# dnbaker/dashing

Measured on AMD Instinct MI355X. Metric: genome-pairs/sec, all-pairs HLL Jaccard (Ertl-MLE), N=10000 p=14, higher is better.
Workload: dtype u8/u32 popcount + f64 estimator; 1 GPU; BASELINE configs[2]: 10000 synthetic sketches, p=14 (16384 B each), all-pairs dist on MI355X; n_sketches=10000, p=14, k=31, estimator=ERTL_MLE

## Files before the change

dashing_amd/csrc/abi.hip:

```cpp
#include <algorithm>
#include <cstdlib>
#include <cstring>
#include <new>

#include "ctx.h"

using namespace dsh;

static hipError_t create_copy_stream(hipStream_t *s)
{
    int least = 0, greatest = 0;
    if (hipDeviceGetStreamPriorityRange(&least, &greatest) != hipSuccess) greatest = 0;
    if (const char *e = std::getenv("DSH_COPY_STREAM_PRIORITY")) greatest = std::atoi(e);
    return hipStreamCreateWithPriority(s, hipStreamNonBlocking, greatest);
}

extern "C" {

const char *dsh_backend_name(void) { return "hip:gfx950"; }

int dsh_abi_version(void) { return DSH_ABI_VERSION; }

int dsh_device_count(void)
{
// ... 1034 lines not shown
#ifdef DSH_WHATIF_MFMA
    if (!std::strcmp(name, "pair_mfma")) {
        c->pair_mfma = v != 0;
        return DSH_OK;
    }
#endif
    if (!std::strcmp(name, "finalize_stop")) {
        if (v < 0 || v > 4) return fail(c, DSH_EINVAL, "finalize_stop must be in [0,4]");
        if (v && !c->profiling) return fail(c, DSH_ESTATE, "finalize_stop needs dsh_set_profiling(ctx, 1)");
        c->finalize_stop = (int)v;
        return DSH_OK;
    }
    if (!std::strcmp(name, "finalize_timing")) {
        if (v && !c->profiling) return fail(c, DSH_ESTATE, "finalize_timing needs dsh_set_profiling(ctx, 1)");
        c->finalize_timing = v != 0;
        return DSH_OK;
    }
    if (!std::strcmp(name, "nsplit")) {
        if (v < 0 || v > 64) return fail(c, DSH_EINVAL, "nsplit must be in [0,64]");
        c->nsplit = (int)v;
        return DSH_OK;
    }
    if (!std::strcmp(name, "emax") || !std::strcmp(name, "elow")) {
        if (v < -1 || v > (int64_t)kMaxListSide) return fail(c, DSH_EINVAL, "%s must be in [-1,%u]", name, kMaxListSide);
        (name[1] == 'm' ? c->emax_opt : c->elow_opt) = (int)v;
        return DSH_OK;
    }
    if (!std::strcmp(name, "part_band_tiles")) {
        if (v < 1 || v > (1 << 30)) return fail(c, DSH_EINVAL, "part_band_tiles out of range");
        c->part_band_tiles = (int)v;
        return DSH_OK;
    }
    if (!std::strcmp(name, "xch_tail_bands")) {
        if (v < 0 || v > 8) return fail(c, DSH_EINVAL, "xch_tail_bands out of range");
        c->tail_bands = (int)v;
        return DSH_OK;
    }
    if (!std::strcmp(name, "overflow_frag_permille")) {
        if (v < 0 || v > 1000) return fail(c, DSH_EINVAL, "overflow_frag_permille out of range");
        c->overflow_frag_permille = (int)v;
        return DSH_OK;
    }
    if (!std::strcmp(name, "xch_recv_gate")) {
        if (v < -1 || v > 1) return fail(c, DSH_EINVAL, "xch_recv_gate is -1 (auto), 0 or 1");
        c->xch_recv_gate = (int)v;
        return DSH_OK;
    }
// ... 10 lines not shown
```

dashing_amd/csrc/consts.h:

```cpp
#pragma once
#include <stdint.h>

namespace dsh {

constexpr uint32_t kTile = 128;
constexpr uint32_t kListCap = 512;
constexpr uint32_t kMaxListSide = 255;
constexpr uint32_t kMaxBuckets = 1u << 15;
constexpr int kMaxPLds = 17;
constexpr int kMaxPReg32 = 15;
constexpr int kMaxPCompare = 24;
constexpr int kMaxP = 24;
constexpr uint32_t kThrChunk = 4096;
constexpr uint32_t kBandMaxRows = 1u << 20;
constexpr uint32_t kSketchSub = 8192;

}
```

dashing_amd/csrc/engine.hip:

```cpp
#include <algorithm>
#include <chrono>
#include <cstring>

#include "ctx.h"

namespace dsh {

int prepare(dsh_ctx *c, int estim, int want_sorted, bool card_only, uint64_t want_rb, uint64_t want_re, uint32_t nparts,
            int rowsorted, const std::vector<uint64_t> *extra_in)
{
    static const std::vector<uint64_t> kNoExtra;
    std::vector<uint64_t> extra_cached;
    const std::vector<uint64_t> *extra = extra_in ? extra_in : &kNoExtra;
    if (!c->have_sketches) return fail(c, DSH_ESTATE, "no sketches loaded");
    if (estim < 0 || estim > 2) return fail(c, DSH_EINVAL, "bad estimator %d", estim);
    if (want_sorted < 0) {
        want_sorted = c->lay.sorted;
        want_rb = c->lay.rb;
        want_re = c->lay.re;
        rowsorted = 0;
        extra_cached = c->lay.extra;
        extra = &extra_cached;
    }
    if (!want_sorted) rowsorted = 0, extra = &kNoExtra;
    if (want_re > c->n) want_re = c->n;
    if (!want_sorted) want_rb = 0, want_re = c->n;
    if (want_rb > want_re) want_rb = want_re;
    const uint64_t n = c->n;
    std::vector<uint64_t> parts, rs_pos;
    if (want_rb >= want_re) extra = &kNoExtra;
    if (want_sorted && !rowsorted) {
        if (extra->empty()) plan::range_parts(n, want_rb, want_re, std::max<uint32_t>(nparts, 1), parts);
        else parts = {want_rb, want_re};
    }
    if (rowsorted) plan::rowsorted_part_positions(n, want_rb, want_re, std::max<uint32_t>(nparts, 1), rs_pos, extra);
    const int emax_new = c->emax_opt >= 0 ? std::min<int>(c->emax_opt, (int)kMaxListSide) : plan::auto_list_cap(c->p, true);
    const int elow_new = c->elow_opt >= 0 ? std::min<int>(c->elow_opt, (int)kMaxListSide) : plan::auto_list_cap(c->p, false);
    if (emax_new != c->emax || elow_new != c->elow) {
        c->planes_valid = false;
        c->card_estim = -1;
    }
    c->emax = emax_new;
    c->elow = elow_new;
    const bool same_layout = c->planes_valid && c->lay_gen == c->pass_gen && c->lay.sorted == want_sorted &&
                             (!want_sorted || (c->lay.rb == want_rb && c->lay.re == want_re && c->lay.rowsorted == rowsorted &&
                                               c->lay.extra == *extra && (rowsorted ? c->lay.part_w == rs_pos : c->lay.parts == parts)));
    const uint64_t need_from = (card_only || !want_sorted || c->pass_from_zero) ? 0 : want_rb;
    const bool have_pass = c->card_estim == estim && c->card_from <= need_from;
    if (have_pass && (card_only || same_layout)) return DSH_OK;
    const bool keep_layout = same_layout && have_pass;
    hipEvent_t e0 = nullptr, e1 = nullptr;
    if (c->profiling) {
        e0 = next_event(c);
        e1 = next_event(c);
        if (e0) (void)hipEventRecord(e0, c->stream);
    }
    if (!have_pass) {
        HIPCHK(c, c->card.ensure(std::max<uint64_t>(n, 1) * sizeof(double)));
        HIPCHK(c, c->exc.ensure(std::max<uint64_t>(n, 1) * kListCap * (c->p <= 15 ? 2 : 4)));
        HIPCHK(c, c->excv.ensure(std::max<uint64_t>(n, 1) * kListCap));
        HIPCHK(c, c->exc_n.ensure(std::max<uint64_t>(n, 1) * sizeof(uint32_t)));
        HIPCHK(c, c->keys.ensure(std::max<uint64_t>(n, 1) * sizeof(uint32_t)));
        HIPCHK(c, c->tailhist.ensure(std::max<uint64_t>(n, 1) * 64));
        HIPCHK(c, c->hist.ensure(std::max<uint64_t>(n, 1) * 64 * sizeof(uint32_t)));
        HIPCHK(c, launch_selfhist_card(c->stream, c->regs, need_from, n, c->p, estim, c->emax, c->elow,
                                       (uint32_t *)c->hist.ptr, c->exc.ptr, (uint8_t *)c->excv.ptr,
                                       (uint32_t *)c->exc_n.ptr, (uint32_t *)c->keys.ptr,
                                       (uint8_t *)c->tailhist.ptr));
        HIPCHK(c, c->pin_keys.ensure(std::max<uint64_t>(n, 1) * sizeof(uint32_t)));
        c->hk32 = (const uint32_t *)c->pin_keys.ptr;
        if (n > need_from)
            HIPCHK(c, hipMemcpyAsync((uint32_t *)c->pin_keys.ptr + need_from, (const uint32_t *)c->keys.ptr + need_from,
                                     (n - need_from) * sizeof(uint32_t), hipMemcpyDeviceToHost, c->stream));
        if (!c->ev_keys) HIPCHK(c, hipEventCreateWithFlags(&c->ev_keys, hipEventDisableTiming));
        HIPCHK(c, hipEventRecord(c->ev_keys, c->stream));
        HIPCHK(c, launch_card_from_hist(c->stream, (const uint32_t *)c->hist.ptr, (const uint32_t *)c->keys.ptr, need_from, n,
                                        c->p, estim, (double *)c->card.ptr));
        c->card_estim = estim;
        c->card_from = need_from;
        c->hk32_valid = false;
        ++c->pass_gen;
    }
    if (card_only) {
// ... 509 lines not shown
```

dashing_amd/csrc/host/plan_capi.cpp:

```cpp
#include <algorithm>
#include <cstdarg>
#include <cstdio>
#include <cstring>
#include <vector>

#include "../plan.h"
#include "../uf.h"

using namespace dsh;
using namespace dsh::plan;

namespace {

struct Err {
    char *buf;
    size_t cap;
    int fail(const char *fmt, ...)
    {
        if (buf && cap) {
            va_list ap;
            va_start(ap, fmt);
            vsnprintf(buf, cap, fmt, ap);
            va_end(ap);
        }
// ... 377 lines not shown
        ++nb;
    }
    return (int64_t)nb;
}

int dsh_plan_uf_labels(uint64_t n, const uint32_t *lhs, const uint32_t *rhs, uint64_t n_edges, uint32_t step_cap, uint32_t *labels_out)
{
    if (n > 0xFFFFFFFFull) return -1;
    std::vector<uint32_t> parent(n);
    for (uint64_t x = 0; x < n; ++x) parent[x] = (uint32_t)x;
    for (uint64_t e = 0; e < n_edges; ++e) {
        if (lhs[e] >= n || rhs[e] >= n) return -1;
        uint32_t why = 0;
        if (uf_unite<UfPlain>(parent.data(), lhs[e], rhs[e], step_cap, &why) == kUfOverrun) return (int)why;
    }
    for (uint64_t x = 0; x < n; ++x) {
        const uint32_t l = uf_find<UfPlain>(parent.data(), (uint32_t)x, step_cap);
        if (l == kUfOverrun) return (int)kUfErrFind;
        labels_out[x] = l;
    }
    return 0;
}

}
```

dashing_amd/csrc/kernels.h:

```cpp
#pragma once
#include <hip/hip_runtime.h>
#include <stdint.h>

#include "consts.h"

namespace dsh {

hipError_t launch_selfhist_card(hipStream_t st, const uint8_t *regs, uint64_t first, uint64_t n, int p, int estim,
                                int emax, int elow, uint32_t *hist, void *exc, uint8_t *excv, uint32_t *exc_n,
                                uint32_t *keys, uint8_t *tailhist);
hipError_t launch_card_from_hist(hipStream_t st, const uint32_t *hist, const uint32_t *keys, uint64_t first, uint64_t n, int p,
                                 int estim, double *card);
inline int colindex_inline(int p, uint32_t E) { return p <= 12 && E <= 256 ? 7 : 3; }
struct ColIndexLaunch {
    const void *exc;
    const uint8_t *excv;
    const uint32_t *exc_n, *keys;
    const double *card;
    const uint8_t *tailhist;
    const uint32_t *perm;
    uint64_t ncols;
    int p;
    uint32_t nblocks, nbuckets, ent_stride, E;
    uint32_t *rec;
    uint32_t *ent;
    uint32_t *nS, *keyS;
    double *cardS;
    uint8_t *thS;
    uint32_t *rl;
};
hipError_t launch_build_colindex(hipStream_t st, const ColIndexLaunch &c);
hipError_t launch_transform(hipStream_t st, const uint8_t *regs, uint64_t n, int p, int vlo,
                            uint32_t P, uint32_t W, uint32_t Npad, uint32_t *planes,
                            const uint32_t *perm);
hipError_t launch_pair_counts(hipStream_t st, int kc, int cum_bytes, const uint32_t *planes,
                              uint32_t Npad, uint32_t Kpad, uint32_t W, uint32_t P,
// ... 216 lines not shown
```

dashing_amd/csrc/kernels_compare.hip:

```cpp
#include <hip/hip_runtime.h>
#include <stdint.h>

#include <algorithm>

#include "estimators.h"
#include "kernels.h"

namespace dsh {

template <typename PT>
__global__ __launch_bounds__(256, 4) void k_selfhist_card(const uint8_t *__restrict__ regs, uint64_t first,
                                                        uint64_t n, int p, int estim, int emax, int elow,
                                                        uint32_t *__restrict__ hist_out,
                                                        PT *__restrict__ exc,
                                                        uint8_t *__restrict__ excv,
                                                        uint32_t *__restrict__ exc_n,
                                                        uint32_t *__restrict__ keys,
                                                        uint8_t *__restrict__ tailhist)
{
    __shared__ uint32_t hist[4][64];
    __shared__ uint32_t sub[4][8][72];
    __shared__ int thr[4], thrL[4];
    const int tid = threadIdx.x, lane = tid & 63, wave = tid >> 6;
    const uint64_t s = first + (uint64_t)blockIdx.x * 4 + wave;
#pragma unroll
    for (int k = 0; k < 8; ++k) sub[wave][k][lane] = 0;
    __syncthreads();
    const uint64_t m = 1ull << p;
    const uint4 *src = reinterpret_cast<const uint4 *>(regs + (s < n ? s : 0) * m);
    const uint64_t nch = m >> 4;
    constexpr int kRegCache = 16;
    uint4 cache[kRegCache];
#pragma unroll
    for (int k = 0; k < kRegCache; ++k) {
        const uint64_t c = (uint64_t)k * 64 + lane;
// ... 36 lines not shown
        while (lo < 63 && h[lo] == 0) ++lo;
        while (hi > 0 && h[hi] == 0) --hi;
        int T = hi;
        uint32_t cnt = 0;
        while (T > lo && cnt + h[T] <= (uint32_t)emax) {
            cnt += h[T];
            --T;
        }
        int L = lo;
        uint32_t cntl = 0;
        while (L < T && cntl + h[L] <= (uint32_t)elow) {
            cntl += h[L];
            ++L;
        }
        thr[wave] = T;
        thrL[wave] = L;
        exc_n[s] = cnt + cntl;
        keys[s] = ((uint32_t)hi << 18) | ((uint32_t)T << 12) | ((uint32_t)L << 6) | (uint32_t)lo;
    }
    if (s < n && __any(bad != 0) && lane == 0) atomicOr(&keys[s], 0x80000000u);
    __syncthreads();
    if (s >= n) return;
    const uint32_t T = (uint32_t)thr[wave], L = (uint32_t)thrL[wave];
    tailhist[s * 64 + lane] = (uint32_t)lane > T ? (uint8_t)hist[wave][lane] : (uint8_t)0;
    hist_out[s * 64 + lane] = hist[wave][lane];
    if (emax == 0 && elow == 0) return;
    PT *dstp = exc + s * kListCap;
    uint8_t *dstv = excv + s * kListCap;
    const uint32_t trep = (T + 1) * 0x01010101u, lrep = L * 0x01010101u;
    auto hits = [trep, lrep](uint32_t x) -> uint32_t {
        const uint32_t ge = ((x | 0x80808080u) - trep) & 0x80808080u;
        const uint32_t lt = ~((x | 0x80808080u) - lrep) & 0x80808080u;
        return ge | lt;
    };
    uint32_t mine = 0;
#pragma unroll
    for (int k = 0; k < kRegCache; ++k)
        if ((uint64_t)k * 64 + lane < nch) {
            const uint32_t w[4] = {cache[k].x, cache[k].y, cache[k].z, cache[k].w};
#pragma unroll
            for (int q = 0; q < 4; ++q) mine += (uint32_t)__popc(hits(w[q]));
        }
    for (uint64_t c = (uint64_t)kRegCache * 64 + lane; c < nch; c += 64) {
        const uint4 x = src[c];
        mine += (uint32_t)(__popc(hits(x.x)) + __popc(hits(x.y)) + __popc(hits(x.z)) + __popc(hits(x.w)));
    }
    uint32_t slot = mine;
#pragma unroll
    for (int d = 1; d < 64; d <<= 1) {
        const uint32_t o = __shfl_up(slot, d, 64);
        if (lane >= d) slot += o;
    }
    slot -= mine;
    auto emit4 = [&](uint32_t x, uint32_t pos0) {
        uint32_t h = hits(x);
        while (h) {
            const uint32_t b = (uint32_t)__builtin_ctz(h) >> 3;
            h &= h - 1;
            if (slot < kListCap) {
                dstp[slot] = (PT)(pos0 + b);
                dstv[slot] = (uint8_t)((x >> (8 * b)) & 0xFFu);
            }
            ++slot;
        }
    };
#pragma unroll
    for (int k = 0; k < kRegCache; ++k) {
        const uint64_t c = (uint64_t)k * 64 + lane;
        if (c < nch) {
            const uint32_t w[4] = {cache[k].x, cache[k].y, cache[k].z, cache[k].w};
#pragma unroll
            for (int q = 0; q < 4; ++q) emit4(w[q], (uint32_t)(c * 16 + q * 4));
        }
    }
    for (uint64_t c = (uint64_t)kRegCache * 64 + lane; c < nch; c += 64) {
        const uint4 x = src[c];
        emit4(x.x, (uint32_t)(c * 16));
        emit4(x.y, (uint32_t)(c * 16 + 4));
        emit4(x.z, (uint32_t)(c * 16 + 8));
        emit4(x.w, (uint32_t)(c * 16 + 12));
    }
}
// ... 19 lines not shown
__global__ __launch_bounds__(1024) void k_build_colindex(const PT *__restrict__ exc, const uint8_t *__restrict__ excv,
                                                          const uint32_t *__restrict__ exc_n,
                                                          const uint32_t *__restrict__ keys, const double *__restrict__ card,
                                                          const uint8_t *__restrict__ tailhist,
                                                          const uint32_t *__restrict__ perm, uint64_t ncols, int p,
                                                          uint32_t nbuckets, uint32_t ent_stride, uint32_t E,
                                                          uint32_t *__restrict__ rec, uint32_t *__restrict__ ent,
                                                          uint32_t *__restrict__ nS, uint32_t *__restrict__ keyS,
                                                          double *__restrict__ cardS, uint8_t *__restrict__ thS,
                                                          uint32_t *__restrict__ rl)
{
    extern __shared__ __attribute__((aligned(16))) uint32_t cnt[];
    __shared__ uint32_t part[1024];
    __shared__ uint32_t below_s;
    constexpr uint32_t RW = (uint32_t)RK + 1u;
    const uint32_t tid = threadIdx.x, lane = tid & 63u, wave = tid >> 6;
    const uint32_t sh = p > 14 ? (uint32_t)(p - 14) : 0u;
    const uint64_t c0 = (uint64_t)blockIdx.x * kTile;
    const uint32_t G = gridDim.y, g = blockIdx.y;
    const uint32_t nown = nbuckets / G, blo = g * nown;
    for (uint32_t b = tid; b < nown; b += 1024) cnt[b] = 0;
    if (tid == 0) below_s = 0;
    __syncthreads();
    constexpr int kPer = (int)(kListCap / 64);
    constexpr int kSk = (int)(kTile / 16);
    uint32_t Ts[kSk], pk[kSk][kPer];
    uint32_t sk[kSk], nes[kSk];
#pragma unroll
    for (int q = 0; q < kSk; ++q) {
        const uint64_t col = c0 + wave + 16u * (uint32_t)q;
        sk[q] = col < ncols ? (perm ? perm[col] : (uint32_t)col) : 0xFFFFFFFFu;
    }
#pragma unroll
    for (int q = 0; q < kSk; ++q) {
        nes[q] = sk[q] != 0xFFFFFFFFu ? exc_n[sk[q]] : 0u;
        Ts[q] = keys[sk[q] != 0xFFFFFFFFu ? sk[q] : 0u];
    }
#pragma unroll
    for (int q = 0; q < kSk; ++q) {
        const uint32_t sl = wave + 16u * (uint32_t)q;
        const bool ok = sk[q] != 0xFFFFFFFFu;
        const uint64_t s = ok ? sk[q] : 0;
        const uint32_t ne = nes[q];
        const uint32_t key = Ts[q];
        Ts[q] = (key >> 12) & 63u;
        const PT *ps = exc + s * kListCap;
        const uint8_t *vs = excv + s * kListCap;
        const uint64_t col = c0 + sl;
        const bool mine = (uint32_t)q % G == g;
        if (mine && lane == 0) {
            nS[col] = ne;
            keyS[col] = ok ? key : 0u;
            cardS[col] = ok ? card[s] : 0.;
        }
        if (mine && lane < 16) reinterpret_cast<uint32_t *>(thS + col * 64)[lane] = ok ? reinterpret_cast<const uint32_t *>(tailhist + s * 64)[lane] : 0u;
        uint32_t pos[kPer], val[kPer];
#pragma unroll
        for (int u = 0; u < kPer; ++u) {
            pos[u] = (uint32_t)ps[lane + 64u * (uint32_t)u];
            val[u] = (uint32_t)vs[lane + 64u * (uint32_t)u];
        }
#pragma unroll
        for (int u = 0; u < kPer; ++u) {
            const uint32_t e = lane + 64u * (uint32_t)u;
            pk[q][u] = e < ne ? ((pos[u] << 8) | val[u]) : 0xFFFFFFFFu;
            if (e < E && mine) rl[col * E + e] = pk[q][u];
        }
        __builtin_amdgcn_sched_barrier(0);
    }
    auto bucket_of = [sh](uint32_t x, uint32_t T) -> uint32_t {
        return x == 0xFFFFFFFFu ? x : ((((x >> 8) >> sh) << 1) | ((x & 0xFFu) > T ? 0u : 1u));
    };
    uint32_t below = 0;
#pragma unroll
    for (int q = 0; q < kSk; ++q)
#pragma unroll
        for (int u = 0; u < kPer; ++u) {
            const uint32_t b = bucket_of(pk[q][u], Ts[q]);
            const uint32_t rel = b - blo;
            if (rel < nown) atomicAdd(&cnt[rel], 1u);
            else if (b < blo) ++below;
        }
    if (G > 1) {
#pragma unroll
        for (int d = 32; d >= 1; d >>= 1) below += __shfl_xor(below, d, 64);
        if (lane == 0 && below) atomicAdd(&below_s, below);
    }
    __syncthreads();
    const uint32_t per = (nown + 1023) / 1024;
    uint32_t sum = 0;
    for (uint32_t b = tid * per; b < (tid + 1) * per && b < nown; ++b) sum += cnt[b];
    uint32_t incl = sum;
#pragma unroll
    for (int d = 1; d < 64; d <<= 1) {
        const uint32_t o = __shfl_up(incl, d, 64);
        if ((int)lane >= d) incl += o;
    }
    if (lane == 63) part[wave] = incl;
    __syncthreads();
    uint32_t wbase = 0;
    for (uint32_t w = 0; w < wave; ++w) wbase += part[w];
    uint32_t run = below_s + wbase + incl - sum;
    uint32_t *myrec = rec + ((uint64_t)blockIdx.x * nbuckets + blo) * RW;
    for (uint32_t b = tid * per; b < (tid + 1) * per && b < nown; ++b) {
        const uint32_t x = cnt[b];
        uint4 *r4 = reinterpret_cast<uint4 *>(myrec + (uint64_t)b * RW);
        r4[0] = make_uint4(x | (run << 16), 0xFFFFFFFFu, 0xFFFFFFFFu, 0xFFFFFFFFu);
        if constexpr (RK > 3) r4[1] = make_uint4(0xFFFFFFFFu, 0xFFFFFFFFu, 0xFFFFFFFFu, 0xFFFFFFFFu);
        cnt[b] = (run << 16) | run;
        run += x;
    }
    __syncthreads();
    uint32_t *myent = ent + (uint64_t)blockIdx.x * ent_stride;
#pragma unroll
    for (int q = 0; q < kSk; ++q)
#pragma unroll
        for (int u = 0; u < kPer; ++u)
        {
            uint32_t x = pk[q][u];
            asm volatile("" : "+v"(x));
            const uint32_t b = bucket_of(x, Ts[q]) - blo;
            if (b < nown) {
                const uint32_t pv = ((((x >> 8) & ((1u << sh) - 1u)) << 13) | ((wave + 16u * (uint32_t)q) << 6) | (x & 0xFFu));
                const uint32_t w = atomicAdd(&cnt[b], 1u);
                const uint32_t slot = w & 0xFFFFu, rel = slot - (w >> 16);
                myent[slot] = pv;
                if (rel < (uint32_t)RK) myrec[(uint64_t)b * RW + 1u + rel] = pv;
            }
        }
}

__device__ __forceinline__ uint32_t lt_word(const uint32_t (&y)[8], uint32_t vrep)
{
    uint32_t ge = 0;
#pragma unroll
    for (int k = 0; k < 8; ++k) ge |= ((y[k] - vrep) >> (7 - k)) & (0x01010101u << k);
    return ~ge;
}

__global__ __launch_bounds__(256) void k_transform(const uint8_t *__restrict__ regs, uint64_t n,
                                                    int p, int vlo, uint32_t P, uint32_t W,
                                                    uint32_t Npad, uint32_t *__restrict__ planes,
                                                    const uint32_t *__restrict__ perm)
{
    const uint64_t gid = (uint64_t)blockIdx.x * 256 + threadIdx.x;
    const uint32_t i = (uint32_t)(gid % Npad);
    const uint32_t w = (uint32_t)(gid / Npad);
    if (w >= W) return;
    const uint64_t m = 1ull << p;
    uint32_t x[8];
#pragma unroll
    for (int k = 0; k < 8; ++k) x[k] = 0xFFFFFFFFu;
// ... 503 lines not shown
{
    unsigned long long tph[7] = {0, 0, 0, 0, 0, 0, 0};
    if constexpr (TIMED) tph[0] = __builtin_readcyclecounter();
    extern __shared__ __attribute__((aligned(16))) unsigned char hs_raw[];
    uint32_t *histA = reinterpret_cast<uint32_t *>(hs_raw);
    uint32_t *corr = histA + 64;
    uint32_t *actm = corr + 128;
    CT *hs = reinterpret_cast<CT *>(hs_raw + (64 + 128 + 8) * 4);
    constexpr uint32_t RW = (uint32_t)RK + 1u;
    constexpr uint32_t kNone = 0xFFFFFFFFu;
    const int tid = threadIdx.x;
    const uint32_t kq = blockIdx.x >> 3;
    const uint32_t tidx = ((kq >> 7) << 3) + (blockIdx.x & 7u), trow = kq & 127u;
    if (tidx >= a.ntiles) return;
    uint4 tile = a.tiles[tidx];
    const int vlo = (int)((tile.z >> 16) & 0xFFu), vhi = (int)(tile.z >> 24);
    const uint32_t slot = ((tile.w & 0xFFFFu) * 128u + trow) * 128u + (uint32_t)tid;
    tile.w = (tile.z >> 8) & 0xFFu;
    tile.z &= 0xFFu;
    const uint32_t si = tile.x * kTile + trow;
    const uint32_t sj = tile.y * kTile + (uint32_t)tid;
    if (si >= a.ncols) return;
    const int Lp = a.pbase + (int)tile.z, T = a.pbase + (int)tile.w;
    constexpr int kR = RK > 3 ? 2 : (int)(kListCap / 128);
    const int nr = (int)((a.E + 127u) >> 7);
    uint32_t le[kR];
    {
        const uint32_t *rli = a.rl + (uint64_t)si * a.E;
#pragma unroll
        for (int r = 0; r < kR; ++r) {
            le[r] = kNone;
            if (r >= nr) continue;
            const uint32_t e = (uint32_t)tid + 128u * (uint32_t)r;
            if (e < a.E) le[r] = rli[e];
        }
    }
    const uint32_t i = a.perm ? (uint32_t)__builtin_amdgcn_readfirstlane((int)a.perm[si]) : si;
    const bool col_ok = sj < a.ncols;
    const uint32_t j = col_ok ? (a.perm ? a.perm[sj] : sj) : 0u;
    const CT *cum0 = reinterpret_cast<const CT *>(a.cum);
    constexpr int kBatch = 16;
    const int npl = (int)(tile.w - tile.z);
    uint32_t cvv[kBatch];
    const int w0 = (T + 1) >> 4;
    uint4 tq[3];
    {
        const CT *cp = cum0 + (uint64_t)tile.z * a.nslots;
#pragma unroll
        for (int t = 0; t < kBatch; ++t) {
            cvv[t] = 0u;
            if (t < npl) {
                cvv[t] = (uint32_t)cp[slot];
                cp += a.nslots;
                asm volatile("" : "+s"(cp));
            }
        }
    }
    {
        const uint4 *tb = reinterpret_cast<const uint4 *>(a.thS) + (sj << 2);
#pragma unroll
        for (int k = 0; k < 3; ++k) tq[k] = w0 + k < 4 ? tb[w0 + k] : make_uint4(0, 0, 0, 0);
    }
    const uint32_t keyj = a.keyS[sj];
    const uint32_t keyi = (uint32_t)__builtin_amdgcn_readfirstlane((int)a.keyS[si]);
    const uint32_t hrow = tid < 64 ? (uint32_t)(a.thS + (uint64_t)si * 64)[tid] : 0u;
    const uint32_t sh = a.p > 14 ? (uint32_t)(a.p - 14) : 0u;
    const uint32_t *brec = a.cidx_rec + (uint64_t)tile.y * a.nbuckets * RW;
    const uint32_t *bent = a.cidx_ent + (uint64_t)tile.y * a.ent_stride;
    const uint32_t rb32 = (uint32_t)a.row_begin, re32 = (uint32_t)a.row_end;
    const bool m_rect = GENERAL && a.rect, m_square = GENERAL && a.square, m_sorted = GENERAL && a.sorted_out, m_knn = GENERAL && a.knn;
    if (m_rect && !(i >= rb32 && i < re32)) return;
    corr[tid] = 0;
    if (tid < 64) histA[tid] = tid > T ? hrow : 0u;
    {
        uint32_t nup = 0;
#pragma unroll
        for (int r = 0; r < kR; ++r) {
            if (r >= nr) break;
            nup += (uint32_t)__popcll(__ballot(le[r] != kNone && (int)(le[r] & 0xFFu) > T));
        }
        if ((tid & 63) == 0) actm[4 + (tid >> 6)] = nup;
    }
    uint32_t oi = i, oj = j;
    bool active;
    if (m_rect) {
        active = j >= (uint32_t)a.col_begin && j < (uint32_t)a.col_end;
    } else if (m_square) {
        active = si < sj;
    } else if (m_sorted || m_knn) {
        oi = si;
        oj = sj;
// ... 36 lines not shown
                prev = cvv[t];
            }
        }
        for (uint32_t pl = tile.z + kBatch; pl < tile.w; ++pl) {
            const uint32_t cv = (cum0 + (uint64_t)pl * a.nslots)[slot];
            dcol[pl * 128] = (CT)(cv - prev);
            prev = cv;
        }
    }
    uint4 rc[kR], rc2[RK > 3 ? kR : 1];
#pragma unroll
    for (int r = 0; r < kR; ++r) {
        rc[r] = make_uint4(0u, kNone, kNone, kNone);
        if constexpr (RK > 3) rc2[r] = make_uint4(kNone, kNone, kNone, kNone);
        if (r >= nr) continue;
        const int va = (int)(le[r] & 0xFFu);
        const bool up = va > T;
        if (le[r] == kNone || !(up || va < Lp)) continue;
        const uint32_t bk = (((le[r] >> 8) >> sh) << 1) | (up ? 0u : 1u);
        const uint4 *rp = reinterpret_cast<const uint4 *>(brec + (uint64_t)bk * RW);
        rc[r] = rp[0];
        if constexpr (RK > 3) rc2[r] = rp[1];
    }
    if (active) {
        const uint32_t qw[12] = {tq[0].x, tq[0].y, tq[0].z, tq[0].w, tq[1].x, tq[1].y, tq[1].z, tq[1].w,
                                 tq[2].x, tq[2].y, tq[2].z, tq[2].w};
        const int x0 = w0 * 16;
        CT *dst = col + (x0 - vlo) * 128;
        const uint32_t *hA = histA + x0;
#pragma unroll
        for (int s_ = 0; s_ < 48; ++s_) {
            const int x = x0 + s_;
            if (x > vhi) break;
            if (x <= T) continue;
            const uint32_t qj = (qw[s_ >> 2] >> (8 * (s_ & 3))) & 0xFFu;
            nb += qj;
            dst[s_ * 128] = (CT)(hA[s_] + qj);
        }
        for (int x = x0 + 48; x <= vhi; ++x) {
            const uint32_t qj = a.thS[(uint64_t)sj * 64 + x];
            nb += qj;
            col[(x - vlo) * 128] = (CT)(histA[x] + qj);
        }
    }
    __syncthreads();
    if constexpr (TIMED) tph[2] = __builtin_readcyclecounter();
    if (a.stop == 2) {
        const FinalizeArgs *L = &a;
        if (active) L->out[out_index(L)] = (float)(nb + prev + keyj);
        return;
    }
    {
        uint32_t *hw = reinterpret_cast<uint32_t *>(hs);
        const bool all_own = (actm[0] & actm[1] & actm[2] & actm[3]) == 0xFFFFFFFFu;
        auto apply = [&](uint32_t x, int var, bool upr, uint32_t plow) {
            const uint32_t jl = (x >> 6) & 127u;
            const int vb = (int)(x & 63u);
            if (x == kNone || (sh && (x >> 13) != plow) || !(upr ? vb > T : vb < Lp)) return;
            if (!all_own && !((actm[jl >> 5] >> (jl & 31u)) & 1u)) return;
            const int bin = upr ? (var < vb ? var : vb) : (var > vb ? var : vb);
            const uint32_t cell = (uint32_t)(bin - vlo) * 128u + jl;
            const uint32_t one = sizeof(CT) == 2 ? 1u << (16u * (cell & 1u)) : 1u;
            uint32_t *w = &hw[sizeof(CT) == 2 ? cell >> 1 : cell];
            if (upr) {
                atomicAdd(&corr[jl], 1u);
                atomicSub(w, one);
            } else {
                atomicAdd(w, one);
            }
        };
#pragma unroll
        for (int r = 0; r < kR; ++r) {
            if (r >= nr) break;
            if (__ballot(rc[r].y != kNone) == 0) continue;
            const int va = (int)(le[r] & 0xFFu);
            const bool up = va > T;
            const uint32_t plow = (le[r] >> 8) & ((1u << sh) - 1u);
            apply(rc[r].y, va, up, plow);
            apply(rc[r].z, va, up, plow);
            apply(rc[r].w, va, up, plow);
            if constexpr (RK > 3) {
                apply(rc2[r].x, va, up, plow);
                apply(rc2[r].y, va, up, plow);
                apply(rc2[r].z, va, up, plow);
                apply(rc2[r].w, va, up, plow);
            }
            const uint32_t cnt = rc[r].x & 0xFFFFu, q0 = rc[r].x >> 16;
            for (uint32_t q = (uint32_t)RK; q < cnt; ++q) apply(bent[q0 + q], va, up, plow);
        }
    }
    __syncthreads();
    if constexpr (TIMED) tph[3] = __builtin_readcyclecounter();
    if (!active) return;
    const uint32_t ucnt = actm[4] + actm[5] + nb - corr[tid];
    uint32_t clow = 0;
    for (int x = vlo; x < Lp; ++x) clow += col[(x - vlo) * 128];
    if (tile.w > tile.z) col[(Lp - vlo) * 128] -= (CT)clow;
    else prev = clow;
    col[(T - vlo) * 128] = (CT)(m - ucnt - prev);
    if (a.stop == 3) {
        const FinalizeArgs *L = &a;
        L->out[out_index(L)] = (float)(ucnt + clow);
        return;
    }
    const int loj = (int)(keyj & 63u), loi = (int)(keyi & 63u);
    const int minv = loi > loj ? loi : loj;
    const int maxj = (int)((keyj >> 18) & 63u), maxi = (int)((keyi >> 18) & 63u);
    int maxv = maxi > maxj ? maxi : maxj;
    if (maxv < T) maxv = T;
    auto c = [col, vlo, vhi](int v) -> uint32_t {
        return (v < vlo || v > vhi) ? 0u : col[(v - vlo) * 128];
// ... 405 lines not shown
    uint64_t most = 0;
    for (uint32_t i = 0; i < nseg; ++i) most = std::max(most, u.s[i].nwords);
    if (!nseg || !most) return hipSuccess;
    const uint32_t blocks = (uint32_t)std::min<uint64_t>(256, (most + 255) / 256);
    hipLaunchKernelGGL(k_upload_segs, dim3(blocks, nseg), dim3(256), 0, st, u);
    return hipGetLastError();
}

hipError_t launch_upload(hipStream_t st, void *dst, const void *src_pinned, size_t bytes)
{
    if (bytes == 0) return hipSuccess;
    const uint64_t nwords = (bytes + 3) / 4;
    const uint32_t blocks = (uint32_t)std::min<uint64_t>(256, (nwords + 255) / 256);
    hipLaunchKernelGGL(k_upload, dim3(blocks), dim3(256), 0, st, (uint32_t *)dst, (const uint32_t *)src_pinned, nwords);
    return hipGetLastError();
}

hipError_t launch_selfhist_card(hipStream_t st, const uint8_t *regs, uint64_t first, uint64_t n, int p, int estim,
                                int emax, int elow, uint32_t *hist, void *exc, uint8_t *excv, uint32_t *exc_n,
                                uint32_t *keys, uint8_t *tailhist)
{
    if (n <= first) return hipSuccess;
    const uint32_t blocks = (uint32_t)((n - first + 3) / 4);
    if (p <= 15)
        hipLaunchKernelGGL(k_selfhist_card<uint16_t>, dim3(blocks), dim3(256), 0, st, regs, first, n, p, estim, emax, elow,
                           hist, (uint16_t *)exc, excv, exc_n, keys, tailhist);
    else
        hipLaunchKernelGGL(k_selfhist_card<uint32_t>, dim3(blocks), dim3(256), 0, st, regs, first, n, p, estim, emax, elow,
                           hist, (uint32_t *)exc, excv, exc_n, keys, tailhist);
    return hipGetLastError();
}

hipError_t launch_card_from_hist(hipStream_t st, const uint32_t *hist, const uint32_t *keys, uint64_t first, uint64_t n, int p,
                                 int estim, double *card)
{
    if (n <= first) return hipSuccess;
    hipLaunchKernelGGL(k_card_from_hist, dim3((uint32_t)((n - first + 63) / 64)), dim3(64), 0, st, hist, keys, first, n, p, estim, card);
    return hipGetLastError();
}

hipError_t launch_build_colindex(hipStream_t st, const ColIndexLaunch &c)
{
    if (c.nblocks == 0) return hipSuccess;
    uint32_t G = 1;
    while (G < 4 && c.nblocks * G < 256 && c.nbuckets / (2 * G) >= 4096) G *= 2;
    const size_t lds = (size_t)(c.nbuckets / G) * sizeof(uint32_t);
#define DSH_COLINDEX(PT, RK)                                                                                                  \
    do {                                                                                                                      \
        hipError_t e = ensure_dynamic_lds(reinterpret_cast<const void *>(k_build_colindex<PT, RK>), lds);                     \
        if (e != hipSuccess) return e;                                                                                        \
        hipLaunchKernelGGL((k_build_colindex<PT, RK>), dim3(c.nblocks, G), dim3(1024), lds, st, (const PT *)c.exc, c.excv,    \
// ... 145 lines not shown
```

dashing_amd/csrc/plan.cpp:

```cpp
#include "plan.h"

#include <algorithm>
#include <cstring>

namespace dsh {
namespace plan {

uint64_t tri_index(uint64_t n, uint64_t i, uint64_t j) { return i * (2 * n - i - 1) / 2 + j - (i + 1); }

uint64_t tri_span(uint64_t n, uint64_t rb, uint64_t re)
{
    if (re > n) re = n;
    if (rb >= re) return 0;
    const uint64_t cnt = re - rb;
    return cnt * (n - 1) - (rb + re - 1) * cnt / 2;
}

uint64_t tri_band_end(uint64_t n, uint64_t b0, uint64_t re, uint64_t band_floats, uint64_t row_cap)
{
    const uint64_t max_rows = std::min<uint64_t>(std::max<uint64_t>(row_cap, 1), kBandMaxRows);
    uint64_t b1 = b0, span = 0;
    do {
        span += n - 1 - b1;
        ++b1;
// ... 72 lines not shown

void range_parts(uint64_t n, uint64_t rb, uint64_t re, uint32_t nparts, std::vector<uint64_t> &out)
{
    out.assign(1, rb);
    if (re > n) re = n;
    if (rb > re) rb = re, out[0] = rb;
    const uint64_t total = tri_span(n, rb, re);
    for (uint32_t q = 1; q < nparts && out.back() < re; ++q) {
        const long double target = (long double)total * q / nparts;
        uint64_t best = out.back() + kTile;
        for (uint64_t cand = out.back() + kTile; cand < re; cand += kTile) {
            best = cand;
            if ((long double)tri_span(n, rb, cand) >= target) break;
        }
        if (best >= re) break;
        out.push_back(best);
    }
    if (out.back() != re) out.push_back(re);
}

int auto_list_cap(int p, bool upper)
{
    const uint64_t m = 1ull << p;
    return (int)std::min<uint64_t>(upper ? kMaxListSide : 200, m >> 5);
}

bool rowsorted_rule(uint64_t n, uint64_t rb, uint64_t re, uint32_t nparts)
{
    if (re > n) re = n;
    if (nparts < 2 || rb >= re) return false;
    return re - rb < (uint64_t)1024 * nparts && tri_span(n, rb, re) * sizeof(float) <= ((uint64_t)1 << 30);
}

uint64_t rowsorted_split(uint64_t n, uint64_t rb, uint64_t re)
{
    if (re > n) re = n;
    if (rb >= re) return re;
    const uint64_t TR = (re - rb + kTile - 1) / kTile, NTc = (n - rb + kTile - 1) / kTile;
    if (TR < 16) return re;
    uint64_t total = 0;
    for (uint64_t t = 0; t < TR; ++t) total += NTc - t;
    uint64_t K = 0, acc = 0;
    while (K < TR && acc * 100 < total * 15) acc += NTc - (TR - 1 - K), ++K;
    if (K < 2 || TR - K < 8) return re;
    const uint64_t x = rb + (TR - K) * kTile;
    const long double len_all = (long double)n - 1 - 0.5L * (long double)(rb + re - 1), len_tail = (long double)n - 1 - 0.5L * (long double)(x + re - 1);
    return len_tail <= 0.65L * len_all ? x : re;
// ... 830 lines not shown
```

Baseline: 3.924 billion pairs/s.

## Allow longer exception lists with chunked column-index build and extended tail histogram

Raises the upper exception-list cap (auto 312 at p=14, up to 1023 by option), sizing per-sketch list storage in 512-entry chunks. The column-index build streams extra chunks from global memory, and the compare kernel software-pipelines the extra rounds. The tail histogram packs overflow counts above 255 into its last bytes. The intent is to cover more pairs exactly through the sparse list path so fewer fall back to the dense slow path. In exchange each pair does more per-pair list work, memory use grows, and the count/offset bit packing changes.

```diff
diff --git a/dashing_amd/csrc/abi.hip b/dashing_amd/csrc/abi.hip
--- a/dashing_amd/csrc/abi.hip
+++ b/dashing_amd/csrc/abi.hip
@@ -1080,7 +1080,8 @@
         return DSH_OK;
     }
     if (!std::strcmp(name, "emax") || !std::strcmp(name, "elow")) {
-        if (v < -1 || v > (int64_t)kMaxListSide) return fail(c, DSH_EINVAL, "%s must be in [-1,%u]", name, kMaxListSide);
+        const uint32_t lim = name[1] == 'm' ? kMaxListUpper : kMaxListLower;
+        if (v < -1 || v > (int64_t)lim) return fail(c, DSH_EINVAL, "%s must be in [-1,%u]", name, lim);
         (name[1] == 'm' ? c->emax_opt : c->elow_opt) = (int)v;
         return DSH_OK;
     }
diff --git a/dashing_amd/csrc/consts.h b/dashing_amd/csrc/consts.h
--- a/dashing_amd/csrc/consts.h
+++ b/dashing_amd/csrc/consts.h
@@ -4,8 +4,11 @@
 namespace dsh {
 
 constexpr uint32_t kTile = 128;
-constexpr uint32_t kListCap = 512;
-constexpr uint32_t kMaxListSide = 255;
+constexpr uint32_t kListChunk = 512;
+constexpr uint32_t kMaxListUpper = 1023;
+constexpr uint32_t kMaxListLower = 255;
+constexpr int kMaxPLongList = 20;
+constexpr uint32_t list_cap(uint32_t E) { return E <= kListChunk ? kListChunk : (E + kListChunk - 1) / kListChunk * kListChunk; }
 constexpr uint32_t kMaxBuckets = 1u << 15;
 constexpr int kMaxPLds = 17;
 constexpr int kMaxPReg32 = 15;
diff --git a/dashing_amd/csrc/engine.hip b/dashing_amd/csrc/engine.hip
--- a/dashing_amd/csrc/engine.hip
+++ b/dashing_amd/csrc/engine.hip
@@ -34,8 +34,9 @@
         else parts = {want_rb, want_re};
     }
     if (rowsorted) plan::rowsorted_part_positions(n, want_rb, want_re, std::max<uint32_t>(nparts, 1), rs_pos, extra);
-    const int emax_new = c->emax_opt >= 0 ? std::min<int>(c->emax_opt, (int)kMaxListSide) : plan::auto_list_cap(c->p, true);
-    const int elow_new = c->elow_opt >= 0 ? std::min<int>(c->elow_opt, (int)kMaxListSide) : plan::auto_list_cap(c->p, false);
+    const int emax_lim = c->p <= kMaxPLongList ? (int)kMaxListUpper : 255;
+    const int emax_new = std::min<int>(c->emax_opt >= 0 ? c->emax_opt : plan::auto_list_cap(c->p, true), emax_lim);
+    const int elow_new = c->elow_opt >= 0 ? std::min<int>(c->elow_opt, (int)kMaxListLower) : plan::auto_list_cap(c->p, false);
     if (emax_new != c->emax || elow_new != c->elow) {
         c->planes_valid = false;
         c->card_estim = -1;
@@ -57,8 +58,9 @@
     }
     if (!have_pass) {
         HIPCHK(c, c->card.ensure(std::max<uint64_t>(n, 1) * sizeof(double)));
-        HIPCHK(c, c->exc.ensure(std::max<uint64_t>(n, 1) * kListCap * (c->p <= 15 ? 2 : 4)));
-        HIPCHK(c, c->excv.ensure(std::max<uint64_t>(n, 1) * kListCap));
+        const uint64_t lcap = list_cap((uint32_t)(c->emax + c->elow));
+        HIPCHK(c, c->exc.ensure(std::max<uint64_t>(n, 1) * lcap * (c->p <= 15 ? 2 : 4)));
+        HIPCHK(c, c->excv.ensure(std::max<uint64_t>(n, 1) * lcap));
         HIPCHK(c, c->exc_n.ensure(std::max<uint64_t>(n, 1) * sizeof(uint32_t)));
         HIPCHK(c, c->keys.ensure(std::max<uint64_t>(n, 1) * sizeof(uint32_t)));
         HIPCHK(c, c->tailhist.ensure(std::max<uint64_t>(n, 1) * 64));
diff --git a/dashing_amd/csrc/host/plan_capi.cpp b/dashing_amd/csrc/host/plan_capi.cpp
--- a/dashing_amd/csrc/host/plan_capi.cpp
+++ b/dashing_amd/csrc/host/plan_capi.cpp
@@ -423,4 +423,6 @@
     return 0;
 }
 
-}
+int dshh_auto_list_cap(int p, int upper) { return dsh::plan::auto_list_cap(p, upper != 0); }
+
+}
diff --git a/dashing_amd/csrc/kernels.h b/dashing_amd/csrc/kernels.h
--- a/dashing_amd/csrc/kernels.h
+++ b/dashing_amd/csrc/kernels.h
@@ -12,6 +12,8 @@
 hipError_t launch_card_from_hist(hipStream_t st, const uint32_t *hist, const uint32_t *keys, uint64_t first, uint64_t n, int p,
                                  int estim, double *card);
 inline int colindex_inline(int p, uint32_t E) { return p <= 12 && E <= 256 ? 7 : 3; }
+constexpr uint32_t cidx_count_bits(int p) { return p <= kMaxPLongList ? 14u : 16u; }
+constexpr int kTailExtMinP = 9;
 struct ColIndexLaunch {
     const void *exc;
     const uint8_t *excv;
diff --git a/dashing_amd/csrc/kernels_compare.hip b/dashing_amd/csrc/kernels_compare.hip
--- a/dashing_amd/csrc/kernels_compare.hip
+++ b/dashing_amd/csrc/kernels_compare.hip
@@ -2,6 +2,7 @@
 #include <stdint.h>
 
 #include <algorithm>
+#include <type_traits>
 
 #include "estimators.h"
 #include "kernels.h"
@@ -10,7 +11,7 @@
 
 template <typename PT>
 __global__ __launch_bounds__(256, 4) void k_selfhist_card(const uint8_t *__restrict__ regs, uint64_t first,
-                                                        uint64_t n, int p, int estim, int emax, int elow,
+                                                        uint64_t n, int p, int estim, int emax, int elow, uint32_t cap,
                                                         uint32_t *__restrict__ hist_out,
                                                         PT *__restrict__ exc,
                                                         uint8_t *__restrict__ excv,
@@ -93,11 +94,23 @@
     __syncthreads();
     if (s >= n) return;
     const uint32_t T = (uint32_t)thr[wave], L = (uint32_t)thrL[wave];
-    tailhist[s * 64 + lane] = (uint32_t)lane > T ? (uint8_t)hist[wave][lane] : (uint8_t)0;
+    {
+        const uint32_t hv = (uint32_t)lane > T ? hist[wave][lane] : 0u;
+        uint32_t byte = hv & 0xFFu;
+        if (p >= kTailExtMinP) {
+            unsigned long long big = __ballot(hv > 0xFFu);
+            if (lane >= 61) {
+                for (int k = 61; k < lane; ++k) big &= big - 1;
+                const int v = big ? __builtin_ctzll(big) : 0;
+                byte = big ? ((uint32_t)v << 2) | ((hist[wave][v] >> 8) & 3u) : 0u;
+            }
+        }
+        tailhist[s * 64 + lane] = (uint8_t)byte;
+    }
     hist_out[s * 64 + lane] = hist[wave][lane];
     if (emax == 0 && elow == 0) return;
-    PT *dstp = exc + s * kListCap;
-    uint8_t *dstv = excv + s * kListCap;
+    PT *dstp = exc + s * cap;
+    uint8_t *dstv = excv + s * cap;
     const uint32_t trep = (T + 1) * 0x01010101u, lrep = L * 0x01010101u;
     auto hits = [trep, lrep](uint32_t x) -> uint32_t {
         const uint32_t ge = ((x | 0x80808080u) - trep) & 0x80808080u;
@@ -128,7 +141,7 @@
         while (h) {
             const uint32_t b = (uint32_t)__builtin_ctz(h) >> 3;
             h &= h - 1;
-            if (slot < kListCap) {
+            if (slot < cap) {
                 dstp[slot] = (PT)(pos0 + b);
                 dstv[slot] = (uint8_t)((x >> (8 * b)) & 0xFFu);
             }
@@ -194,8 +207,11 @@
     for (uint32_t b = tid; b < nown; b += 1024) cnt[b] = 0;
     if (tid == 0) below_s = 0;
     __syncthreads();
-    constexpr int kPer = (int)(kListCap / 64);
+    constexpr int kPer = (int)(kListChunk / 64);
     constexpr int kSk = (int)(kTile / 16);
+    const uint32_t cap = list_cap(E);
+    const uint32_t nch = cap / kListChunk;
+    const uint32_t cb = cidx_count_bits(p);
     uint32_t Ts[kSk], pk[kSk][kPer];
     uint32_t sk[kSk], nes[kSk];
 #pragma unroll
@@ -208,98 +224,154 @@
         nes[q] = sk[q] != 0xFFFFFFFFu ? exc_n[sk[q]] : 0u;
         Ts[q] = keys[sk[q] != 0xFFFFFFFFu ? sk[q] : 0u];
     }
-#pragma unroll
-    for (int q = 0; q < kSk; ++q) {
-        const uint32_t sl = wave + 16u * (uint32_t)q;
-        const bool ok = sk[q] != 0xFFFFFFFFu;
-        const uint64_t s = ok ? sk[q] : 0;
-        const uint32_t ne = nes[q];
-        const uint32_t key = Ts[q];
-        Ts[q] = (key >> 12) & 63u;
-        const PT *ps = exc + s * kListCap;
-        const uint8_t *vs = excv + s * kListCap;
-        const uint64_t col = c0 + sl;
-        const bool mine = (uint32_t)q % G == g;
-        if (mine && lane == 0) {
-            nS[col] = ne;
-            keyS[col] = ok ? key : 0u;
-            cardS[col] = ok ? card[s] : 0.;
-        }
-        if (mine && lane < 16) reinterpret_cast<uint32_t *>(thS + col * 64)[lane] = ok ? reinterpret_cast<const uint32_t *>(tailhist + s * 64)[lane] : 0u;
-        uint32_t pos[kPer], val[kPer];
-#pragma unroll
-        for (int u = 0; u < kPer; ++u) {
-            pos[u] = (uint32_t)ps[lane + 64u * (uint32_t)u];
-            val[u] = (uint32_t)vs[lane + 64u * (uint32_t)u];
-        }
-#pragma unroll
-        for (int u = 0; u < kPer; ++u) {
-            const uint32_t e = lane + 64u * (uint32_t)u;
-            pk[q][u] = e < ne ? ((pos[u] << 8) | val[u]) : 0xFFFFFFFFu;
-            if (e < E && mine) rl[col * E + e] = pk[q][u];
-        }
-        __builtin_amdgcn_sched_barrier(0);
-    }
+    {
+#pragma unroll
+        for (int q = 0; q < kSk; ++q) {
+            const uint32_t sl = wave + 16u * (uint32_t)q;
+            const bool ok = sk[q] != 0xFFFFFFFFu;
+            const uint64_t s = ok ? sk[q] : 0;
+            const uint32_t ne = nes[q];
+            const uint32_t key = Ts[q];
+            Ts[q] = (key >> 12) & 63u;
+            const PT *ps = exc + s * cap;
+            const uint8_t *vs = excv + s * cap;
+            const uint64_t col = c0 + sl;
+            const bool mine = (uint32_t)q % G == g;
+            if (mine && lane == 0) {
+                nS[col] = ne;
+                keyS[col] = ok ? key : 0u;
+                cardS[col] = ok ? card[s] : 0.;
+            }
+            if (mine && lane < 16) reinterpret_cast<uint32_t *>(thS + col * 64)[lane] = ok ? reinterpret_cast<const uint32_t *>(tailhist + s * 64)[lane] : 0u;
+            uint32_t pos[kPer], val[kPer];
+#pragma unroll
+            for (int u = 0; u < kPer; ++u) {
+                pos[u] = (uint32_t)ps[lane + 64u * (uint32_t)u];
+                val[u] = (uint32_t)vs[lane + 64u * (uint32_t)u];
+            }
+#pragma unroll
+            for (int u = 0; u < kPer; ++u) {
+                const uint32_t e = lane + 64u * (uint32_t)u;
+                pk[q][u] = e < ne ? ((pos[u] << 8) | val[u]) : 0xFFFFFFFFu;
+                if (e < E && mine) rl[col * E + e] = pk[q][u];
+            }
+            __builtin_amdgcn_sched_barrier(0);
+        }
+    }
+    auto stream_chunk = [&](uint32_t ch, auto wrl_c, auto &&use) {
+        constexpr bool kWrl = decltype(wrl_c)::value;
+        uint32_t z = 0;
+        asm volatile("" : "+v"(z));
+        const uint32_t lane = (tid + z) & 63u, wave = (tid + z) >> 6;
+        const uint32_t e0 = ch * kListChunk;
+        auto sketch_of = [&](uint32_t q) -> uint32_t {
+            const uint64_t col = c0 + wave + 16u * q;
+            return q < (uint32_t)kSk && col < ncols ? (perm ? perm[col] : (uint32_t)col) : 0xFFFFFFFFu;
+        };
+        uint32_t sknext = sketch_of(0u);
+#pragma unroll 1
+        for (uint32_t q = 0; q < (uint32_t)kSk; ++q) {
+            const uint32_t skq = sknext;
+            sknext = sketch_of(q + 1u);
+            const uint32_t sl = wave + 16u * q;
+            const bool ok = skq != 0xFFFFFFFFu;
+            const uint64_t s = ok ? skq : 0;
+            const PT *ps = exc + s * cap + e0;
+            const uint8_t *vs = excv + s * cap + e0;
+            const uint64_t col = c0 + sl;
+            const bool mine = q % G == g;
+            const uint32_t ne = ok ? exc_n[s] : 0u;
+            const uint32_t T = (keys[s] >> 12) & 63u;
+            uint32_t pos[kPer], val[kPer];
+#pragma unroll
+            for (int u = 0; u < kPer; ++u) {
+                pos[u] = (uint32_t)ps[lane + 64u * (uint32_t)u];
+                val[u] = (uint32_t)vs[lane + 64u * (uint32_t)u];
+            }
+#pragma unroll
+            for (int u = 0; u < kPer; ++u) {
+                const uint32_t e = e0 + lane + 64u * (uint32_t)u;
+                const uint32_t x = e < ne ? ((pos[u] << 8) | val[u]) : 0xFFFFFFFFu;
+                if constexpr (kWrl)
+                    if (e < E && mine) rl[col * E + e] = x;
+                use(x, T, sl);
+            }
+        }
+    };
+    const std::true_type yes;
+    const std::false_type no;
     auto bucket_of = [sh](uint32_t x, uint32_t T) -> uint32_t {
         return x == 0xFFFFFFFFu ? x : ((((x >> 8) >> sh) << 1) | ((x & 0xFFu) > T ? 0u : 1u));
     };
     uint32_t below = 0;
+    auto count_one = [&](uint32_t x, uint32_t T, uint32_t) {
+        const uint32_t b = bucket_of(x, T);
+        const uint32_t rel = b - blo;
+        if (rel < nown) atomicAdd(&cnt[rel], 1u);
+        else if (b < blo) ++below;
+    };
 #pragma unroll
     for (int q = 0; q < kSk; ++q)
 #pragma unroll
-        for (int u = 0; u < kPer; ++u) {
-            const uint32_t b = bucket_of(pk[q][u], Ts[q]);
-            const uint32_t rel = b - blo;
-            if (rel < nown) atomicAdd(&cnt[rel], 1u);
-            else if (b < blo) ++below;
-        }
-    if (G > 1) {
-#pragma unroll
-        for (int d = 32; d >= 1; d >>= 1) below += __shfl_xor(below, d, 64);
-        if (lane == 0 && below) atomicAdd(&below_s, below);
-    }
-    __syncthreads();
-    const uint32_t per = (nown + 1023) / 1024;
-    uint32_t sum = 0;
-    for (uint32_t b = tid * per; b < (tid + 1) * per && b < nown; ++b) sum += cnt[b];
-    uint32_t incl = sum;
-#pragma unroll
-    for (int d = 1; d < 64; d <<= 1) {
-        const uint32_t o = __shfl_up(incl, d, 64);
-        if ((int)lane >= d) incl += o;
-    }
-    if (lane == 63) part[wave] = incl;
-    __syncthreads();
-    uint32_t wbase = 0;
-    for (uint32_t w = 0; w < wave; ++w) wbase += part[w];
-    uint32_t run = below_s + wbase + incl - sum;
+        for (int u = 0; u < kPer; ++u) count_one(pk[q][u], Ts[q], 0u);
     uint32_t *myrec = rec + ((uint64_t)blockIdx.x * nbuckets + blo) * RW;
-    for (uint32_t b = tid * per; b < (tid + 1) * per && b < nown; ++b) {
-        const uint32_t x = cnt[b];
-        uint4 *r4 = reinterpret_cast<uint4 *>(myrec + (uint64_t)b * RW);
-        r4[0] = make_uint4(x | (run << 16), 0xFFFFFFFFu, 0xFFFFFFFFu, 0xFFFFFFFFu);
-        if constexpr (RK > 3) r4[1] = make_uint4(0xFFFFFFFFu, 0xFFFFFFFFu, 0xFFFFFFFFu, 0xFFFFFFFFu);
-        cnt[b] = (run << 16) | run;
-        run += x;
-    }
-    __syncthreads();
     uint32_t *myent = ent + (uint64_t)blockIdx.x * ent_stride;
-#pragma unroll
-    for (int q = 0; q < kSk; ++q)
-#pragma unroll
-        for (int u = 0; u < kPer; ++u)
-        {
-            uint32_t x = pk[q][u];
-            asm volatile("" : "+v"(x));
-            const uint32_t b = bucket_of(x, Ts[q]) - blo;
-            if (b < nown) {
-                const uint32_t pv = ((((x >> 8) & ((1u << sh) - 1u)) << 13) | ((wave + 16u * (uint32_t)q) << 6) | (x & 0xFFu));
-                const uint32_t w = atomicAdd(&cnt[b], 1u);
-                const uint32_t slot = w & 0xFFFFu, rel = slot - (w >> 16);
-                myent[slot] = pv;
-                if (rel < (uint32_t)RK) myrec[(uint64_t)b * RW + 1u + rel] = pv;
-            }
-        }
+    auto scan_headers = [&]() {
+        if (G > 1) {
+#pragma unroll
+            for (int d = 32; d >= 1; d >>= 1) below += __shfl_xor(below, d, 64);
+            if (lane == 0 && below) atomicAdd(&below_s, below);
+        }
+        __syncthreads();
+        const uint32_t per = (nown + 1023) / 1024;
+        uint32_t sum = 0;
+        for (uint32_t b = tid * per; b < (tid + 1) * per && b < nown; ++b) sum += cnt[b];
+        uint32_t incl = sum;
+#pragma unroll
+        for (int d = 1; d < 64; d <<= 1) {
+            const uint32_t o = __shfl_up(incl, d, 64);
+            if ((int)lane >= d) incl += o;
+        }
+        if (lane == 63) part[wave] = incl;
+        __syncthreads();
+        uint32_t wbase = 0;
+        for (uint32_t w = 0; w < wave; ++w) wbase += part[w];
+        uint32_t run = below_s + wbase + incl - sum;
+        for (uint32_t b = tid * per; b < (tid + 1) * per && b < nown; ++b) {
+            const uint32_t x = cnt[b];
+            uint4 *r4 = reinterpret_cast<uint4 *>(myrec + (uint64_t)b * RW);
+            r4[0] = make_uint4(x | (run << cb), 0xFFFFFFFFu, 0xFFFFFFFFu, 0xFFFFFFFFu);
+            if constexpr (RK > 3) r4[1] = make_uint4(0xFFFFFFFFu, 0xFFFFFFFFu, 0xFFFFFFFFu, 0xFFFFFFFFu);
+            cnt[b] = run << cb;
+            run += x;
+        }
+        __syncthreads();
+    };
+    auto place_one = [&](uint32_t x, uint32_t T, uint32_t sl) {
+        const uint32_t b = bucket_of(x, T) - blo;
+        if (b < nown) {
+            const uint32_t pv = ((((x >> 8) & ((1u << sh) - 1u)) << 13) | (sl << 6) | (x & 0xFFu));
+            const uint32_t w = atomicAdd(&cnt[b], 1u);
+            const uint32_t rel = w & ((1u << cb) - 1u), slot = (w >> cb) + rel;
+            myent[slot] = pv;
+            if (rel < (uint32_t)RK) myrec[(uint64_t)b * RW + 1u + rel] = pv;
+        }
+    };
+    if (nch == 1) {
+        scan_headers();
+#pragma unroll
+        for (int q = 0; q < kSk; ++q)
+#pragma unroll
+            for (int u = 0; u < kPer; ++u) {
+                uint32_t x = pk[q][u];
+                asm volatile("" : "+v"(x));
+                place_one(x, Ts[q], wave + 16u * (uint32_t)q);
+            }
+    } else {
+        for (uint32_t ch = 1; ch < nch; ++ch) stream_chunk(ch, yes, count_one);
+        scan_headers();
+        for (uint32_t ch = 0; ch < nch; ++ch) stream_chunk(ch, no, place_one);
+    }
 }
 
 __device__ __forceinline__ uint32_t lt_word(const uint32_t (&y)[8], uint32_t vrep)
@@ -849,7 +921,9 @@
     const uint32_t sj = tile.y * kTile + (uint32_t)tid;
     if (si >= a.ncols) return;
     const int Lp = a.pbase + (int)tile.z, T = a.pbase + (int)tile.w;
-    constexpr int kR = RK > 3 ? 2 : (int)(kListCap / 128);
+    constexpr int kR = RK > 3 ? 2 : 4;
+    constexpr int kX = 2;
+    constexpr bool kLong = RK == 3;
     const int nr = (int)((a.E + 127u) >> 7);
     uint32_t le[kR];
     {
@@ -862,6 +936,16 @@
             if (e < a.E) le[r] = rli[e];
         }
     }
+    auto load_rounds = [&](int base, uint32_t (&dst)[kX]) {
+        const uint32_t *rli = a.rl + (uint64_t)si * a.E;
+#pragma unroll
+        for (int r = 0; r < kX; ++r) {
+            dst[r] = kNone;
+            if (base + r >= nr) continue;
+            const uint32_t e = (uint32_t)tid + 128u * (uint32_t)(base + r);
+            if (e < a.E) dst[r] = rli[e];
+        }
+    };
     const uint32_t i = a.perm ? (uint32_t)__builtin_amdgcn_readfirstlane((int)a.perm[si]) : si;
     const bool col_ok = sj < a.ncols;
     const uint32_t j = col_ok ? (a.perm ? a.perm[sj] : sj) : 0u;
@@ -890,10 +974,24 @@
     }
     const uint32_t keyj = a.keyS[sj];
     const uint32_t keyi = (uint32_t)__builtin_amdgcn_readfirstlane((int)a.keyS[si]);
-    const uint32_t hrow = tid < 64 ? (uint32_t)(a.thS + (uint64_t)si * 64)[tid] : 0u;
+    uint32_t hrow = tid < 64 ? (uint32_t)(a.thS + (uint64_t)si * 64)[tid] : 0u;
+    const bool th_ext = a.p >= kTailExtMinP && a.E >= 256u;
+    uint32_t extj = 0;
+    if (th_ext) {
+        extj = reinterpret_cast<const uint32_t *>(a.thS)[(sj << 4) + 15u] >> 8;
+        const uint32_t exti = (uint32_t)__builtin_amdgcn_readfirstlane((int)reinterpret_cast<const uint32_t *>(a.thS)[(si << 4) + 15u]) >> 8;
+        if (exti) {
+#pragma unroll
+            for (int k = 0; k < 3; ++k) {
+                const uint32_t e = (exti >> (8 * k)) & 0xFFu;
+                if ((e >> 2) == (uint32_t)tid) hrow += (e & 3u) << 8;
+            }
+        }
+    }
     const uint32_t sh = a.p > 14 ? (uint32_t)(a.p - 14) : 0u;
     const uint32_t *brec = a.cidx_rec + (uint64_t)tile.y * a.nbuckets * RW;
     const uint32_t *bent = a.cidx_ent + (uint64_t)tile.y * a.ent_stride;
+    const uint32_t cb = cidx_count_bits(a.p);
     const uint32_t rb32 = (uint32_t)a.row_begin, re32 = (uint32_t)a.row_end;
     const bool m_rect = GENERAL && a.rect, m_square = GENERAL && a.square, m_sorted = GENERAL && a.sorted_out, m_knn = GENERAL && a.knn;
     if (m_rect && !(i >= rb32 && i < re32)) return;
@@ -976,6 +1074,20 @@
         rc[r] = rp[0];
         if constexpr (RK > 3) rc2[r] = rp[1];
     }
+    auto gather_rounds = [&](const uint32_t (&l)[kX], uint4 (&rcx)[kX]) {
+#pragma unroll
+        for (int r = 0; r < kX; ++r) {
+            rcx[r] = make_uint4(0u, kNone, kNone, kNone);
+            const int va = (int)(l[r] & 0xFFu);
+            const bool up = va > T;
+            if (l[r] == kNone || !(up || va < Lp)) continue;
+            const uint32_t bk = (((l[r] >> 8) >> sh) << 1) | (up ? 0u : 1u);
+            rcx[r] = *reinterpret_cast<const uint4 *>(brec + (uint64_t)bk * RW);
+        }
+    };
+    uint32_t ln[kX] = {kNone, kNone};
+    if constexpr (kLong)
+        if (nr > kR) load_rounds(kR, ln);
     if (active) {
         const uint32_t qw[12] = {tq[0].x, tq[0].y, tq[0].z, tq[0].w, tq[1].x, tq[1].y, tq[1].z, tq[1].w,
                                  tq[2].x, tq[2].y, tq[2].z, tq[2].w};
@@ -995,6 +1107,17 @@
             const uint32_t qj = a.thS[(uint64_t)sj * 64 + x];
             nb += qj;
             col[(x - vlo) * 128] = (CT)(histA[x] + qj);
+        }
+        if (extj) {
+#pragma unroll
+            for (int k = 0; k < 3; ++k) {
+                const uint32_t e = (extj >> (8 * k)) & 0xFFu;
+                const int x = (int)(e >> 2);
+                if (e && x > T && x <= vhi) {
+                    nb += (e & 3u) << 8;
+                    col[(x - vlo) * 128] += (CT)((e & 3u) << 8);
+                }
+            }
         }
     }
     __syncthreads();
@@ -1023,6 +1146,13 @@
                 atomicAdd(w, one);
             }
         };
+        uint4 rn[kX];
+        uint32_t l2[kX] = {kNone, kNone};
+        if constexpr (kLong)
+            if (nr > kR) {
+                gather_rounds(ln, rn);
+                load_rounds(kR + kX, l2);
+            }
 #pragma unroll
         for (int r = 0; r < kR; ++r) {
             if (r >= nr) break;
@@ -1039,8 +1169,33 @@
                 apply(rc2[r].z, va, up, plow);
                 apply(rc2[r].w, va, up, plow);
             }
-            const uint32_t cnt = rc[r].x & 0xFFFFu, q0 = rc[r].x >> 16;
+            const uint32_t cnt = rc[r].x & ((1u << cb) - 1u), q0 = rc[r].x >> cb;
             for (uint32_t q = (uint32_t)RK; q < cnt; ++q) apply(bent[q0 + q], va, up, plow);
+        }
+        if constexpr (kLong) {
+            uint32_t nupx = 0;
+            for (int base = kR; base < nr; base += kX) {
+                uint4 rnn[kX];
+                uint32_t l3[kX];
+                gather_rounds(l2, rnn);
+                load_rounds(base + 2 * kX, l3);
+#pragma unroll
+                for (int r = 0; r < kX; ++r) {
+                    const int va = (int)(ln[r] & 0xFFu);
+                    const bool up = va > T;
+                    nupx += (uint32_t)__popcll(__ballot(ln[r] != kNone && up));
+                    if (__ballot(rn[r].y != kNone) == 0) continue;
+                    const uint32_t plow = (ln[r] >> 8) & ((1u << sh) - 1u);
+                    apply(rn[r].y, va, up, plow);
+                    apply(rn[r].z, va, up, plow);
+                    apply(rn[r].w, va, up, plow);
+                    const uint32_t cnt = rn[r].x & ((1u << cb) - 1u), q0 = rn[r].x >> cb;
+                    for (uint32_t q = (uint32_t)RK; q < cnt; ++q) apply(bent[q0 + q], va, up, plow);
+                }
+#pragma unroll
+                for (int r = 0; r < kX; ++r) ln[r] = l2[r], rn[r] = rnn[r], l2[r] = l3[r];
+            }
+            if (nupx && (tid & 63) == 0) actm[4 + (tid >> 6)] += nupx;
         }
     }
     __syncthreads();
@@ -1492,11 +1647,12 @@
 {
     if (n <= first) return hipSuccess;
     const uint32_t blocks = (uint32_t)((n - first + 3) / 4);
+    const uint32_t cap = list_cap((uint32_t)(emax + elow));
     if (p <= 15)
-        hipLaunchKernelGGL(k_selfhist_card<uint16_t>, dim3(blocks), dim3(256), 0, st, regs, first, n, p, estim, emax, elow,
+        hipLaunchKernelGGL(k_selfhist_card<uint16_t>, dim3(blocks), dim3(256), 0, st, regs, first, n, p, estim, emax, elow, cap,
                            hist, (uint16_t *)exc, excv, exc_n, keys, tailhist);
     else
-        hipLaunchKernelGGL(k_selfhist_card<uint32_t>, dim3(blocks), dim3(256), 0, st, regs, first, n, p, estim, emax, elow,
+        hipLaunchKernelGGL(k_selfhist_card<uint32_t>, dim3(blocks), dim3(256), 0, st, regs, first, n, p, estim, emax, elow, cap,
                            hist, (uint32_t *)exc, excv, exc_n, keys, tailhist);
     return hipGetLastError();
 }
diff --git a/dashing_amd/csrc/plan.cpp b/dashing_amd/csrc/plan.cpp
--- a/dashing_amd/csrc/plan.cpp
+++ b/dashing_amd/csrc/plan.cpp
@@ -118,7 +118,9 @@
 int auto_list_cap(int p, bool upper)
 {
     const uint64_t m = 1ull << p;
-    return (int)std::min<uint64_t>(upper ? kMaxListSide : 200, m >> 5);
+    if (!upper) return (int)std::min<uint64_t>(200, m >> 5);
+    const uint64_t clip = p == 14 ? 312 : (p >= 16 && p <= kMaxPLongList) ? 512 : 255;
+    return (int)std::min<uint64_t>(clip, m >> 5);
 }
 
 bool rowsorted_rule(uint64_t n, uint64_t rb, uint64_t re, uint32_t nparts)
```

Result: no change. 3.912 billion pairs/s (-0.3%).
